# Firstastor/polars-quant

Hardware: AMD Instinct MI355X
Metric: indicator+backtest rows/sec, 5000 sym x 2520 day f64 OHLCV (higher is better)
Workload: dtype f64

## Files before the change

### polars_quant_amd/csrc/fused.hip

```cpp
#include "ops_fused.h"
#include "wt_api.h"

extern "C" {
pq_status pq_trima_chain(pq_ctx *, const pq_batch *, const double *, int64_t, double *);
pq_status pq_cci_chain(pq_ctx *, const pq_batch *, const double *, const double *, const double *, int64_t, double *);
pq_status pq_adxr_chain(pq_ctx *, const pq_batch *, const double *, const double *, const double *, int64_t, double *);
pq_status pq_adxr_from_adx(pq_ctx *, const pq_batch *, const double *, int64_t, double *);
pq_status pq_apo_chain(pq_ctx *, const pq_batch *, const double *, int64_t, int64_t, int64_t, double *);
pq_status pq_ppo_chain(pq_ctx *, const pq_batch *, const double *, int64_t, int64_t, int64_t, double *);
pq_status pq_macdext_chain(pq_ctx *, const pq_batch *, const double *, int64_t, int64_t, int64_t, int64_t, int64_t, int64_t,
                           double *, double *, double *);
pq_status pq_stoch_chain(pq_ctx *, const pq_batch *, const double *, const double *, const double *, int64_t, int64_t,
                         int64_t, int64_t, int64_t, double *, double *);
pq_status pq_stochf_chain(pq_ctx *, const pq_batch *, const double *, const double *, const double *, int64_t, int64_t,
                          int64_t, double *, double *);
pq_status pq_stochrsi_chain(pq_ctx *, const pq_batch *, const double *, int64_t, int64_t, int64_t, int64_t, double *, double *);
}

#define CHK(name, cond) PQ_TRY(pq_check(ctx, b)); PQ_REQUIRE(cond, name ": null pointer")

constexpr int HT_TS_MAX_CHUNKS = 8;
struct HtTsBlob {
    HtAll6Op op;
    const double *real;
// ... 247 lines not shown
    MacdPairOp op{};
    op.a.fast = fast; op.a.slow = slow; op.a.sig = sig; op.b.fast = 12; op.b.slow = 26; op.b.sig = fix_sig;
    InCols<1> in{{real}}; OutCols<6> o{{macd, signal, hist, fmacd, fsignal, fhist}};
    if (PQ_FUSE_OK(ctx) && seq_can_lds(ctx, b, op, in, o)) return launch_seq(ctx, b, op, in, o);
    PQ_TRY(pq_macd(ctx, b, real, fast, slow, sig, macd, signal, hist));
    return pq_macdfix(ctx, b, real, fix_sig, fmacd, fsignal, fhist);
}
pq_status pq_sar_pair(pq_ctx *ctx, const pq_batch *b, const double *high, const double *low, double accel, double maxv, double startvalue,
                      double offsetonreverse, double ai_long, double a_long, double am_long, double ai_short, double a_short,
                      double am_short, double *sar, double *sarext) {
    CHK("pq_sar_pair", high && low && sar && sarext);
    SarPairOp op{};
    op.a.ext = false; op.a.startvalue = 0.0; op.a.offset = 0.0;
    op.a.ai_long = op.a.a_long = op.a.ai_short = op.a.a_short = accel; op.a.am_long = op.a.am_short = maxv;
    op.b.ext = true; op.b.startvalue = startvalue; op.b.offset = offsetonreverse;
    op.b.ai_long = ai_long; op.b.a_long = a_long; op.b.am_long = am_long; op.b.ai_short = ai_short; op.b.a_short = a_short; op.b.am_short = am_short;
    InCols<2> in{{high, low}}; OutCols<2> o{{sar, sarext}};
    if (PQ_FUSE_OK(ctx) && seq_can_lds(ctx, b, op, in, o)) return launch_seq(ctx, b, op, in, o);
    PQ_TRY(pq_sar(ctx, b, high, low, accel, maxv, sar));
    return pq_sarext(ctx, b, high, low, startvalue, offsetonreverse, ai_long, a_long, am_long, ai_short, a_short, am_short, sarext);
}
pq_status pq_volume_all(pq_ctx *ctx, const pq_batch *b, const double *h, const double *l, const double *c, const double *v, int64_t mfi_p,
                        int64_t fast, int64_t slow, double *mfi, double *ad, double *adosc, double *obv) {
    CHK("pq_volume_all", h && l && c && v && mfi && ad && adosc && obv);
    VolumeAllOp op{};
    op.a.p = mfi_p; op.b.a.a.fast = op.b.a.a.slow = 0; op.b.a.b.fast = fast; op.b.a.b.slow = slow;
    InCols<4> in{{h, l, c, v}}; OutCols<4> o{{mfi, ad, adosc, obv}};
    if (PQ_FUSE_OK(ctx) && seq_can_lds(ctx, b, op, in, o)) return launch_seq(ctx, b, op, in, o);
    PQ_TRY(pq_mfi(ctx, b, h, l, c, v, mfi_p, mfi)); PQ_TRY(pq_ad(ctx, b, h, l, c, v, ad));
    PQ_TRY(pq_adosc(ctx, b, h, l, c, v, fast, slow, adosc));
    return pq_obv(ctx, b, c, v, obv);
}
pq_status pq_dm_system_all(pq_ctx *ctx, const pq_batch *b, const double *h, const double *l, const double *c, int64_t p, double *dx,
                           double *plus_di, double *minus_di, double *adx, double *adxr, double *atr, double *natr) {
    CHK("pq_dm_system_all", h && l && c && dx && plus_di && minus_di && adx && adxr && atr && natr);
    {
        pq_status st;
        if (wt_dmi(ctx, b, h, l, c, p, dx, plus_di, minus_di, adx, adxr, &st)) {
            PQ_TRY(st);
            return pq_atr_all(ctx, b, h, l, c, p, atr, natr);
        }
    }
    DmiAtrOp op{}; op.a.p = p; op.b.a.p = p; op.b.b.p = p;
    InCols<3> in{{h, l, c}}; OutCols<7> o{{dx, plus_di, minus_di, adx, adxr, atr, natr}};
    if (PQ_FUSE_OK(ctx) && seq_can_lds(ctx, b, op, in, o)) return launch_seq(ctx, b, op, in, o);
    PQ_TRY(pq_dmi_all(ctx, b, h, l, c, p, dx, plus_di, minus_di, adx, adxr));
    return pq_atr_all(ctx, b, h, l, c, p, atr, natr);
}
pq_status pq_sma_ma(pq_ctx *ctx, const pq_batch *b, const double *real, int64_t p, double *sma, double *ma) {
    CHK("pq_sma_ma", real && sma && ma);
    SmaDupOp op{}; op.a.p = p;
    InCols<1> in{{real}}; OutCols<2> o{{sma, ma}};
    if (PQ_FUSE_OK(ctx) && seq_can_lds(ctx, b, op, in, o)) return launch_seq(ctx, b, op, in, o);
    PQ_TRY(pq_sma(ctx, b, real, p, sma));
    return pq_ma(ctx, b, real, p, 0, ma);
}
pq_status pq_cmo_rsi(pq_ctx *ctx, const pq_batch *b, const double *real, int64_t p, double *cmo, double *rsi) {
    CHK("pq_cmo_rsi", real && cmo && rsi);
    {
        pq_status st;
        if (wt_rsi(ctx, b, real, p, rsi, &st)) { PQ_TRY(st); return pq_cmo(ctx, b, real, p, cmo); }
    }
    CmoRsiOp op{}; op.a.p = p; op.b.p = p;
    InCols<1> in{{real}}; OutCols<2> o{{cmo, rsi}};
    if (PQ_FUSE_OK(ctx) && seq_can_lds(ctx, b, op, in, o)) return launch_seq(ctx, b, op, in, o);
    PQ_TRY(pq_cmo(ctx, b, real, p, cmo));
    return pq_rsi(ctx, b, real, p, rsi);
}
pq_status pq_stoch_all(pq_ctx *ctx, const pq_batch *b, const double *h, const double *l, const double *c, int64_t fastk, int64_t slowk,
                       int64_t slowk_mt, int64_t slowd, int64_t slowd_mt, int64_t fastd, int64_t fastd_mt, double *slowk_out,
                       double *slowd_out, double *fastk_out, double *fastd_out) {
    CHK("pq_stoch_all", h && l && c && slowk_out && slowd_out && fastk_out && fastd_out);
    StochAllOp op{};
    op.fastk = fastk; op.slowk = slowk; op.slowk_mt = slowk_mt; op.slowd = slowd; op.slowd_mt = slowd_mt; op.fastd = fastd; op.fastd_mt = fastd_mt;
    InCols<3> in{{h, l, c}}; OutCols<4> o{{slowk_out, slowd_out, fastk_out, fastd_out}};
    if (PQ_FUSE_OK(ctx) && Ma2::supports(slowk_mt) && Ma2::supports(slowd_mt) && Ma2::supports(fastd_mt) && seq_can_lds(ctx, b, op, in, o))
        return launch_seq(ctx, b, op, in, o);
    PQ_TRY(pq_stoch(ctx, b, h, l, c, fastk, slowk, slowk_mt, slowd, slowd_mt, slowk_out, slowd_out));
    return pq_stochf(ctx, b, h, l, c, fastk, fastd, fastd_mt, fastk_out, fastd_out);
}
pq_status pq_apo_ppo(pq_ctx *ctx, const pq_batch *b, const double *real, int64_t fast, int64_t slow, int64_t matype, double *apo, double *ppo) {
    CHK("pq_apo_ppo", real && apo && ppo);
    ApoPpoOp op{};
    op.a.fast = fast; op.a.slow = slow; op.a.matype = matype; op.b.fast = fast; op.b.slow = slow; op.b.matype = matype;
    InCols<1> in{{real}}; OutCols<2> o{{apo, ppo}};
    if (PQ_FUSE_OK(ctx) && Ma2::supports(matype) && seq_can_lds(ctx, b, op, in, o)) return launch_seq(ctx, b, op, in, o);
    PQ_TRY(pq_apo(ctx, b, real, fast, slow, matype, apo));
    return pq_ppo(ctx, b, real, fast, slow, matype, ppo);
}

}
```

### polars_quant_amd/csrc/ops_fused.h

```cpp
#pragma once
#include "ops_misc.h"
#include "ops_momentum.h"
#include "ops_overlap.h"

struct Ma2 {
    int kind;
    int dead;
    int64_t p, count;
    double k;
    double acc;
    Ring w;
    __host__ __device__ static bool supports(int64_t matype) { return !(matype >= 2 && matype <= 6) && matype != 8; }
    __host__ __device__ static int64_t slots(int64_t matype, int64_t p) { return matype == 1 ? 0 : (p > 0 ? p : 1); }
    __device__ __forceinline__ void init_core(int kind_, int64_t p_, int64_t n) {
        kind = kind_;
        p = p_;
        dead = (p <= 0 || n < p) ? 1 : 0;
        k = pq_uniform(kind ? 2.0 / ((double)p + 1.0) : 1.0 / (double)p);
        count = 0;
        acc = 0.0;
    }
    __device__ __forceinline__ void init(int64_t matype, int64_t p_, int64_t n, RingAlloc &ra) {
        init_core(matype == 1 ? 1 : 0, p_, n);
        if (!kind) w = ra.make(p_);
    }
    __device__ __forceinline__ bool steady() const { return !dead && count >= p; }
    __device__ __forceinline__ double step_old(double v, double old) {
        if (wave_all(!dead && count >= p && !pq_isnull(v))) {
            acc += v;
            acc -= old;
            return acc * k;
        }
        if (dead || pq_isnull(v)) return pq_null();
        count += 1;
        acc += v;
        if (count < p) return pq_null();
        if (count > p) {
            acc -= old;
            count -= 1;
        }
        return acc * k;
    }
    __device__ __forceinline__ double fast_old(double v, double old) {
        acc += v;
        acc -= old;
        return acc * k;
    }
    __device__ __forceinline__ double step(double v) {
        if (!kind) {
            if (wave_all(!dead && count >= p && !pq_isnull(v))) {
                acc += v;
                acc -= w.swap(v);
                return acc * k;
            }
            if (dead || pq_isnull(v)) return pq_null();
            count += 1;
            acc += v;
            const double old = w.swap(v);
            if (count < p) return pq_null();
            if (count > p) {
                acc -= old;
                count -= 1;
            }
            return acc * k;
        }
        if (wave_all(!dead && count >= p && !pq_isnull(v))) {
            acc = fma(k, v - acc, acc);
            return acc;
        }
        if (dead || pq_isnull(v)) return pq_null();
        count += 1;
        if (count < p) {
            acc += v;
            return pq_null();
        } else if (count == p) {
            acc += v;
            acc = acc / (double)p;
            return acc;
        }
        acc = fma(k, v - acc, acc);
        return acc;
    }
    __device__ __forceinline__ double fast(double v) {
        if (!kind) {
            acc += v;
            acc -= w.swap(v);
            return acc * k;
        }
        acc = fma(k, v - acc, acc);
        return acc;
    }
};

struct Ma2Pair {
    Ma2 a, b;
    Ring w;
    bool shared;
    int pa, pb;
    __host__ __device__ static int64_t slots(int64_t mta, int64_t pa_, int64_t mtb, int64_t pb_) {
        if (mta != 1 && mtb != 1) { int64_t m = pa_ > pb_ ? pa_ : pb_; return m > 0 ? m : 1; }
        return Ma2::slots(mta, pa_) + Ma2::slots(mtb, pb_);
    }
    __device__ __forceinline__ void init(int64_t mta, int64_t pa_, int64_t mtb, int64_t pb_, int64_t n, RingAlloc &ra) {
        shared = (mta != 1 && mtb != 1);
        if (shared) {
            a.init_core(0, pa_, n); b.init_core(0, pb_, n);
            pa = (int)(pa_ > 0 ? pa_ : 1); pb = (int)(pb_ > 0 ? pb_ : 1);
            w = ra.make(pa_ > pb_ ? pa_ : pb_);
            asm volatile("" ::: "memory");
        } else {
            a.init(mta, pa_, n, ra); b.init(mtb, pb_, n, ra);
        }
    }
    __device__ __forceinline__ void step(double v, double &ya, double &yb) {
        if (!shared) { ya = a.step(v); yb = b.step(v); return; }
        if (pq_isnull(v)) { ya = yb = pq_null(); return; }
        const double oa = w.get(pa), ob = w.get(pb);
        ya = a.step_old(v, oa);
        yb = b.step_old(v, ob);
        w.push(v);
    }
    __device__ __forceinline__ bool steady() const { return a.steady() && b.steady(); }
    __device__ __forceinline__ void fast(double v, double &ya, double &yb) {
        if (!shared) { ya = a.fast(v); yb = b.fast(v); return; }
        const double oa = w.get(pa), ob = w.get(pb);
        ya = a.fast_old(v, oa);
        yb = b.fast_old(v, ob);
        w.push(v);
    }
};

struct TrimaOp {
    static constexpr bool LDS_ONLY = true;
    static constexpr int NIN = 1, NOUT = 1;
    static constexpr int SEQ_ID = 70;
    static constexpr int COST_NS = 150;
    int64_t k1, k2;
    SmaCore a, b;
    Ring wa, wb;
    __host__ __device__ int64_t ring_slots() const { return (k1 > 0 ? k1 : 1) + (k2 > 0 ? k2 : 1); }
    __device__ void init(const Row<1> &) {}
    __device__ void init_lds(const Row<1> &r, RingAlloc &ra) { a.init(k1, r.len); b.init(k2, r.len); wa = ra.make(k1); wb = ra.make(k2); }
    __device__ void step(const Row<1> &, int64_t, const double (&)[1], double (&y)[1]) { y[0] = pq_null(); }
    __device__ void step_lds(int64_t, const double (&x)[1], double (&y)[1]) { y[0] = b.step_ring(wb, a.step_ring(wa, x[0])); }
    static constexpr bool HAS_FAST = true;
    __device__ bool steady(int64_t) const { return a.steady() && b.steady(); }
    __device__ void step_fast(int64_t, const double (&x)[1], double (&y)[1]) { y[0] = b.fast_ring(wb, a.fast_ring(wa, x[0])); }
};

struct SmaDupOp {
    static constexpr bool LDS_ONLY = true;
    static constexpr int NIN = 1, NOUT = 2;
    static constexpr int SEQ_ID = 88;
    static constexpr int ASSIST = 1;
    static constexpr int ALG_COLS = 4;
    static constexpr int COST_NS = 130;
    SmaOp a;
    __host__ __device__ int64_t ring_slots() const { return a.ring_slots(); }
    __device__ void init(const Row<1> &) {}
    __device__ void init_lds(const Row<1> &r, RingAlloc &ra) { a.init_lds(r, ra); }
    __device__ void step(const Row<1> &, int64_t, const double (&)[1], double (&y)[2]) { y[0] = y[1] = pq_null(); }
    __device__ void step_lds(int64_t t, const double (&x)[1], double (&y)[2]) { double v[1]; a.step_lds(t, x, v); y[0] = y[1] = v[0]; }
    static constexpr bool HAS_FAST = true;
    __device__ bool steady(int64_t t0) const { return a.steady(t0); }
    __device__ void step_fast(int64_t t, const double (&x)[1], double (&y)[2]) { double v[1]; a.step_fast(t, x, v); y[0] = y[1] = v[0]; }
    static constexpr bool FAST_BATCH = true;
    static constexpr int FAST_UNROLL = 8;
    template <int N>
    __device__ void steps_fast(int64_t t, const double (&x)[N][1], double (&y)[N][2]) {
        double v[N][1];
        a.template steps_fast<N>(t, x, v);
#pragma unroll
        for (int u = 0; u < N; u++) y[u][0] = y[u][1] = v[u][0];
    }
};

template <int MODE>
struct MaDiffOp {
    static constexpr bool LDS_ONLY = true;
    static constexpr int NIN = 1, NOUT = 1;
    static constexpr int SEQ_ID = 71 + MODE;
    static constexpr int COST_NS = 500;
    int64_t fast, slow, matype;
    Ma2Pair fs;
    __host__ __device__ int64_t ring_slots() const { return Ma2Pair::slots(matype, fast, matype, slow); }
    __device__ void init(const Row<1> &) {}
    __device__ void init_lds(const Row<1> &r, RingAlloc &ra) { fs.init(matype, fast, matype, slow, r.len, ra); }
    __device__ void step(const Row<1> &, int64_t, const double (&)[1], double (&y)[1]) { y[0] = pq_null(); }
    __device__ void step_lds(int64_t, const double (&x)[1], double (&y)[1]) {
        double a, b;
        fs.step(x[0], a, b);
        if (pq_isnull(a) || pq_isnull(b)) { y[0] = pq_null(); return; }
        if (MODE == 0) y[0] = a - b;
        else y[0] = (b == 0.0) ? pq_null() : (a - b) / b * 100.0;
    }
    static constexpr bool HAS_FAST = true;
    __device__ bool steady(int64_t) const { return fs.steady(); }
    __device__ void step_fast(int64_t, const double (&x)[1], double (&y)[1]) {
        double a, b;
        fs.fast(x[0], a, b);
        if (MODE == 0) y[0] = a - b;
        else { const double v = (a - b) / b * 100.0; y[0] = (b == 0.0) ? pq_null() : v; }
    }
};

struct MacdextOp {
    static constexpr bool LDS_ONLY = true;
    static constexpr int NIN = 1, NOUT = 3;
    static constexpr int SEQ_ID = 73;
    static constexpr int COST_NS = 338;
    int64_t fast, fastmt, slow, slowmt, sig, sigmt;
    Ma2Pair fs;
    Ma2 g;
    __host__ __device__ int64_t ring_slots() const { return Ma2Pair::slots(fastmt, fast, slowmt, slow) + Ma2::slots(sigmt, sig); }
    __device__ __forceinline__ void init(const Row<1> &) {}
    __device__ __forceinline__ void init_lds(const Row<1> &r, RingAlloc &ra) {
        fs.init(fastmt, fast, slowmt, slow, r.len, ra); g.init(sigmt, sig, r.len, ra);
    }
    __device__ __forceinline__ void step(const Row<1> &, int64_t, const double (&)[1], double (&y)[3]) { y[0] = y[1] = y[2] = pq_null(); }
    __device__ __forceinline__ void step_lds(int64_t, const double (&x)[1], double (&y)[3]) {
        double a, b;
        fs.step(x[0], a, b);
        double m = (pq_isnull(a) || pq_isnull(b)) ? pq_null() : a - b;
        double d = g.step(m);
        y[0] = m; y[1] = d;
        y[2] = (pq_isnull(m) || pq_isnull(d)) ? pq_null() : m - d;
    }
    static constexpr bool HAS_FAST = true;
    __device__ __forceinline__ bool steady(int64_t) const { return fs.steady() && g.steady(); }
    __device__ __forceinline__ void step_fast(int64_t, const double (&x)[1], double (&y)[3]) {
        double a, b;
        fs.fast(x[0], a, b);
        const double m = a - b;
        const double d = g.fast(m);
        y[0] = m; y[1] = d; y[2] = m - d;
    }
};

struct FastkCore {
    int64_t k, rows, nulls_h, nulls_l;
    Ring nh, nl;
    RollExt<true> mx;
    RollExt<false> mn;
    Ring hc, hs, lc, ls;
    __host__ __device__ static int64_t slots(int64_t k) { return 6 * (k > 0 ? k : 1); }
    __device__ void init(int64_t k_, RingAlloc &ra) {
        k = k_; rows = 0; nulls_h = nulls_l = 0;
        nh = ra.make(k); nl = ra.make(k);
        mx.init(k); mn.init(k); mx.init_ring(); mn.init_ring();
        hc = ra.make(k); hs = ra.make(k); lc = ra.make(k); ls = ra.make(k);
    }
    __device__ double step(double h, double l, double c) {
        if (k <= 0) return pq_null();
        const bool hn_ = pq_isnull(h), ln_ = pq_isnull(l);
        double oh = nh.swap(hn_ ? 1.0 : 0.0), ol = nl.swap(ln_ ? 1.0 : 0.0);
        if (rows >= k) { nulls_h -= (oh != 0.0) ? 1 : 0; nulls_l -= (ol != 0.0) ? 1 : 0; }
        nulls_h += hn_ ? 1 : 0; nulls_l += ln_ ? 1 : 0;
        rows += 1;
        double hmax = mx.step_ring2(hc, hs, hn_ ? -1.7976931348623157e308 : h);
        double lmin = mn.step_ring2(lc, ls, ln_ ? 1.7976931348623157e308 : l);
        if (rows < k || nulls_h || nulls_l || pq_isnull(c)) return pq_null();
        return (c - lmin) * 100.0 / (hmax - lmin);
    }
    __device__ bool steady() const { return k > 0 && rows >= k && nulls_h == 0 && nulls_l == 0; }
    __device__ double fast(double h, double l, double c) {
        const double hmax = mx.step_ring2(hc, hs, h);
        const double lmin = mn.step_ring2(lc, ls, l);
        return (c - lmin) * 100.0 / (hmax - lmin);
    }
};

template <int MODE>
struct StochOp {
    static constexpr bool RG_GATHER = true;
    static constexpr int64_t DIRECT_LANE_MAX = 16384;
    static constexpr bool LDS_ONLY = true;
    static constexpr int NIN = 3, NOUT = 2;
    static constexpr int SEQ_ID = 74 + MODE;
    static constexpr int COST_NS = MODE == 0 ? 637 : 579;
    static constexpr bool HEAVY = false;
    int64_t fastk, p1, mt1, p2, mt2;
    FastkCore fk;
    Ma2 m1, m2;
    __host__ __device__ int64_t ring_slots() const {
        return FastkCore::slots(fastk) + Ma2::slots(mt1, p1) + (MODE == 0 ? Ma2::slots(mt2, p2) : 0);
    }
    __device__ void init(const Row<3> &) {}
    __device__ void init_lds(const Row<3> &r, RingAlloc &ra) {
        fk.init(fastk, ra);
        m1.init(mt1, p1, r.len, ra);
        if (MODE == 0) m2.init(mt2, p2, r.len, ra);
    }
    __device__ void step(const Row<3> &, int64_t, const double (&)[3], double (&y)[2]) { y[0] = y[1] = pq_null(); }
    __device__ void step_lds(int64_t, const double (&x)[3], double (&y)[2]) {
        double k = fk.step(x[0], x[1], x[2]);
        double a = m1.step(k);
        if (MODE == 0) { y[0] = a; y[1] = m2.step(a); }
        else { y[0] = k; y[1] = a; }
    }
    static constexpr bool HAS_FAST = true;
    __device__ bool steady(int64_t) const { return fk.steady() && m1.steady() && (MODE != 0 || m2.steady()); }
    __device__ void step_fast(int64_t, const double (&x)[3], double (&y)[2]) {
        const double k = fk.fast(x[0], x[1], x[2]);
        const double a = m1.fast(k);
        if (MODE == 0) { y[0] = a; y[1] = m2.fast(a); }
        else { y[0] = k; y[1] = a; }
    }
};

struct StochAllOp {
    static constexpr bool RG_GATHER = true;
    static constexpr bool LDS_ONLY = true;
    static constexpr int NIN = 3, NOUT = 4;
    static constexpr int ALG_COLS = 5 + 5;
    static constexpr int SEQ_ID = 96;
    static constexpr int COST_NS = 800;
    int64_t fastk, slowk, slowk_mt, slowd, slowd_mt, fastd, fastd_mt;
    FastkCore fk;
    Ma2 mk, md, mf;
    __host__ __device__ int64_t ring_slots() const {
        return FastkCore::slots(fastk) + Ma2::slots(slowk_mt, slowk) + Ma2::slots(slowd_mt, slowd) + Ma2::slots(fastd_mt, fastd);
    }
    __device__ void init(const Row<3> &) {}
    __device__ void init_lds(const Row<3> &r, RingAlloc &ra) {
        fk.init(fastk, ra);
        mk.init(slowk_mt, slowk, r.len, ra); md.init(slowd_mt, slowd, r.len, ra); mf.init(fastd_mt, fastd, r.len, ra);
    }
    __device__ void step(const Row<3> &, int64_t, const double (&)[3], double (&y)[4]) { y[0] = y[1] = y[2] = y[3] = pq_null(); }
    __device__ void step_lds(int64_t, const double (&x)[3], double (&y)[4]) {
        const double k = fk.step(x[0], x[1], x[2]);
        const double a = mk.step(k);
        y[0] = a; y[1] = md.step(a); y[2] = k; y[3] = mf.step(k);
    }
    static constexpr bool HAS_FAST = true;
    __device__ bool steady(int64_t) const { return fk.steady() && mk.steady() && md.steady() && mf.steady(); }
    __device__ void step_fast(int64_t, const double (&x)[3], double (&y)[4]) {
        const double k = fk.fast(x[0], x[1], x[2]);
        const double a = mk.fast(k);
        y[0] = a; y[1] = md.fast(a); y[2] = k; y[3] = mf.fast(k);
    }
};

struct StochRsiOp {
    static constexpr bool RG_GATHER = true;
    static constexpr int64_t DIRECT_LANE_MAX = 16384;
    static constexpr bool LDS_ONLY = true;
    static constexpr int NIN = 1, NOUT = 2;
    static constexpr int SEQ_ID = 76;
    static constexpr int COST_NS = 618;
    int64_t p, fastk, fastd, fastd_mt;
    RsiOp rsi;
    FastkCore fk;
    Ma2 m;
    __host__ __device__ int64_t ring_slots() const { return FastkCore::slots(fastk) + Ma2::slots(fastd_mt, fastd); }
    __device__ void init(const Row<1> &) {}
    __device__ void init_lds(const Row<1> &r, RingAlloc &ra) { rsi.p = p; rsi.init(r); fk.init(fastk, ra); m.init(fastd_mt, fastd, r.len, ra); }
    __device__ void step(const Row<1> &, int64_t, const double (&)[1], double (&y)[2]) { y[0] = y[1] = pq_null(); }
    __device__ void step_lds(int64_t i, const double (&x)[1], double (&y)[2]) {
        double rv[1];
        Row<1> dummy; dummy.in[0] = nullptr; dummy.len = 0;
        rsi.step(dummy, i, x, rv);
        double k = fk.step(rv[0], rv[0], rv[0]);
        y[0] = k;
        y[1] = m.step(k);
    }
    static constexpr bool FAST_NULL_OK = true;
    static constexpr bool HAS_FAST = true;
    __device__ bool steady(int64_t t0) const { return rsi.steady(t0) && fk.steady() && m.steady(); }
    __device__ void step_fast(int64_t i, const double (&x)[1], double (&y)[2]) {
        double rv[1];
        rsi.step_fast(i, x, rv);
        const double k = fk.fast(rv[0], rv[0], rv[0]);
        y[0] = k;
        y[1] = m.fast(k);
    }
};

struct CciOp {
    static constexpr bool LDS_ONLY = true;
    static constexpr int NIN = 3, NOUT = 1;
    static constexpr int SEQ_ID = 77;
    __host__ int cost_ns() const { return 320 + 40 * (int)(p > 0 ? (p < 1000 ? p : 1000) : 0); }
    int64_t p;
    double sum, denom;
    bool dead;
    Ring w;
    __host__ __device__ int64_t ring_slots() const { return p > 0 ? p : 1; }
    __device__ void init(const Row<3> &) {}
    __device__ void init_lds(const Row<3> &r, RingAlloc &ra) {
        dead = (p <= 0 || r.len < p); sum = 0.0; denom = 1.0 / (double)p; w = ra.make(p);
    }
    __device__ void step(const Row<3> &, int64_t, const double (&)[3], double (&y)[1]) { y[0] = pq_null(); }
    __device__ void step_lds(int64_t i, const double (&x)[3], double (&y)[1]) {
        y[0] = pq_null();
        if (dead) return;
        double tp = (x[0] + x[1] + x[2]) / 3.0;
        sum += tp;
        double old = w.swap(tp);
        if (i < p - 1) return;
        if (i >= p) sum -= old;
        double avg = sum * denom;
        double mean_dev = 0.0;
        for (int b0 = (int)p; b0 >= 1; b0 -= 8) {
            double v8[8];
            w.get8<-1>(b0, v8);
#pragma unroll
            for (int u = 0; u < 8; u++)
                if (b0 - u >= 1) mean_dev += fabs(v8[u] - avg);
        }
        if (mean_dev != 0.0) {
            mean_dev /= (double)p;
            y[0] = (tp - avg) / (0.015 * mean_dev);
        }
    }
    static constexpr bool FAST_NULL_OK = true;
    static constexpr bool HAS_FAST = true;
    __device__ bool steady(int64_t t0) const { return !dead && t0 >= p; }
    __device__ void step_fast(int64_t, const double (&x)[3], double (&y)[1]) {
        const double tp = (x[0] + x[1] + x[2]) / 3.0;
        sum += tp;
        sum -= w.swap(tp);
        const double avg = sum * denom;
        double mean_dev = 0.0;
        for (int b0 = (int)p; b0 >= 1; b0 -= 8) {
            double v8[8];
            w.get8<-1>(b0, v8);
#pragma unroll
            for (int u = 0; u < 8; u++)
                if (b0 - u >= 1) mean_dev += fabs(v8[u] - avg);
        }
        const double md = mean_dev / (double)p;
        const double v = (tp - avg) / (0.015 * md);
        y[0] = (mean_dev != 0.0) ? v : pq_null();
    }
    static constexpr bool FAST_BATCH = true;
    static constexpr int FAST_UNROLL = 8;
    template <int N>
    __device__ void steps_fast(int64_t, const double (&x)[N][3], double (&y)[N][1]) {
        static_assert(N == 8, "CciOp::steps_fast is written for batches of eight rows");
        double tp[8], old[8], avg[8], md[8];
#pragma unroll
        for (int r = 0; r < 8; r++) tp[r] = (x[r][0] + x[r][1] + x[r][2]) / 3.0;
        w.swap_n<8>(tp, old);
#pragma unroll
        for (int r = 0; r < 8; r++) {
            sum += tp[r];
            sum -= old[r];
            avg[r] = sum * denom;
            md[r] = 0.0;
        }
        double W[15];
#pragma unroll
        for (int i = 0; i < 7; i++) W[i] = old[i + 1];
        int k = w.pos;
        const int ip = (int)p;
        for (int b0 = 0; b0 < ip; b0 += 8) {
#pragma unroll
// ... 432 lines not shown
template <int ID, class A, class B>
struct Fuse2 {
    static_assert(A::NIN == B::NIN, "fused ops must read the same input columns");
    static_assert(!IsMasked<A>::value && !IsMasked<B>::value && !HasFinish<A>::value && !HasFinish<B>::value, "not fusable");
    static_assert(NTap<A>::value == 0 || HasRings<A>::value, "tap-only ops cannot be fused");
    static_assert(NTap<B>::value == 0 || HasRings<B>::value, "tap-only ops cannot be fused");
    static constexpr int NIN = A::NIN, NOUT = A::NOUT + B::NOUT;
    static constexpr int ALG_COLS = AlgCols<A>::value + AlgCols<B>::value;
    static constexpr int SEQ_ID = ID;
    static constexpr int ASSIST = FuseAssist<ID>::value;
    __host__ int cost_ns() const { return (3 * (OpCost<A>::get(a) + OpCost<B>::get(b))) / 4; }
    static constexpr bool HEAVY = IsHeavy<A>::value || IsHeavy<B>::value;
    static constexpr bool LDS_ONLY = true;
    A a;
    B b;
    __host__ __device__ int64_t ring_slots() const {
        int64_t n = 0;
        if constexpr (HasRings<A>::value) n += a.ring_slots();
        if constexpr (HasRings<B>::value) n += b.ring_slots();
        return n;
    }
    __device__ void init(const Row<NIN> &) {}
    __device__ void init_lds(const Row<NIN> &r, RingAlloc &ra) {
        if constexpr (HasRings<A>::value) a.init_lds(r, ra); else a.init(r);
        if constexpr (HasRings<B>::value) b.init_lds(r, ra); else b.init(r);
        row = r;
    }
    Row<NIN> row;
    __device__ void step(const Row<NIN> &, int64_t, const double (&)[NIN], double (&y)[NOUT]) {
#pragma unroll
        for (int k = 0; k < NOUT; k++) y[k] = pq_null();
    }
    __device__ void step_lds(int64_t t, const double (&x)[NIN], double (&y)[NOUT]) {
        double ya[A::NOUT], yb[B::NOUT];
        if constexpr (HasRings<A>::value) a.step_lds(t, x, ya); else a.step(row, t, x, ya);
        if constexpr (HasRings<B>::value) b.step_lds(t, x, yb); else b.step(row, t, x, yb);
#pragma unroll
        for (int k = 0; k < A::NOUT; k++) y[k] = ya[k];
#pragma unroll
        for (int k = 0; k < B::NOUT; k++) y[A::NOUT + k] = yb[k];
    }
    static constexpr bool FAST_NULL_OK = FastNullOk<A>::value && FastNullOk<B>::value;
    static constexpr int FAST_UNROLL = FastUnroll<A>::value < FastUnroll<B>::value ? FastUnroll<A>::value : FastUnroll<B>::value;
    static constexpr bool HAS_FAST = HasFast<A>::value && HasFast<B>::value;
    __device__ bool steady(int64_t t0) const { return a.steady(t0) && b.steady(t0); }
    __device__ void step_fast(int64_t t, const double (&x)[NIN], double (&y)[NOUT]) {
        double ya[A::NOUT], yb[B::NOUT];
        a.step_fast(t, x, ya);
        b.step_fast(t, x, yb);
#pragma unroll
        for (int k = 0; k < A::NOUT; k++) y[k] = ya[k];
#pragma unroll
        for (int k = 0; k < B::NOUT; k++) y[A::NOUT + k] = yb[k];
    }
};

template <int NIN_, class Op, int I0, int I1>
struct Pick2 {
    static_assert(Op::NIN == 2 && !HasRings<Op>::value && NTap<Op>::value == 0, "Pick2 wraps a plain two-input op");
    static constexpr int NIN = NIN_, NOUT = Op::NOUT;
    static constexpr int ALG_COLS = AlgCols<Op>::value;
    static constexpr int COST_NS = OpCostStatic<Op>::value;
    Op op;
    Row<2> rr;
    __device__ void init(const Row<NIN> &r) { rr.in[0] = r.in[I0]; rr.in[1] = r.in[I1]; rr.len = r.len; op.init(rr); }
    __device__ void step(const Row<NIN> &, int64_t t, const double (&x)[NIN], double (&y)[NOUT]) {
        const double xx[2] = {x[I0], x[I1]};
        op.step(rr, t, xx, y);
    }
    static constexpr bool FAST_NULL_OK = FastNullOk<Op>::value;
    static constexpr bool HAS_FAST = HasFast<Op>::value;
    __device__ bool steady(int64_t t0) const { return op.steady(t0); }
    __device__ void step_fast(int64_t t, const double (&x)[NIN], double (&y)[NOUT]) {
        const double xx[2] = {x[I0], x[I1]};
        op.step_fast(t, xx, y);
    }
};

typedef Fuse2<90, Fuse2<0, EmaOp, DemaOp>, Fuse2<0, TemaOp, TrixOp>> EmaAllOp;
typedef Fuse2<91, AtrOp<false>, AtrOp<true>> AtrAllOp;
typedef Fuse2<92, DmRawOp<true>, DmRawOp<false>> DmPairOp;
typedef Fuse2<93, AdOp<false>, AdOp<true>> AdAllOp;
typedef Fuse2<94, MacdOp, MacdOp> MacdPairOp;
typedef Fuse2<95, MaDiffOp<0>, MaDiffOp<1>> ApoPpoOp;
typedef Fuse2<97, SarextOp, SarextOp> SarPairOp;
typedef Fuse2<99, DmAllOp<true>, AtrAllOp> DmiAtrOp;
typedef Fuse2<89, CmoOp, RsiOp> CmoRsiOp;
typedef Fuse2<98, MfiOp, Fuse2<0, AdAllOp, Pick2<4, ObvOp, 2, 3>>> VolumeAllOp;
```

### polars_quant_amd/csrc/ops_overlap.h

```cpp
#pragma once
#include "pq_cores.h"

struct SmaOp {
    static constexpr int NIN = 1, NOUT = 1;
    static constexpr int SEQ_ID = 1;
    static constexpr int COST_NS = 116;
    static constexpr int NTAP = 1;
    static constexpr int TAP_COL[1] = {0};
    int64_t p;
    SmaCore c;
    __device__ void init(const Row<1> &r) { c.init(p, r.len); }
    __device__ void tap_lags(int64_t (&lag)[1]) const { lag[0] = c.dead ? 0 : p; }
    __device__ void step(const Row<1> &r, int64_t t, const double (&x)[1], const double (&tp)[1], double (&y)[1]) {
        y[0] = c.step(r.in[0], t, x[0], tp[0]);
    }
    Ring w;
    __host__ __device__ int64_t ring_slots() const { return p > 0 ? p : 1; }
    __device__ void init_lds(const Row<1> &r, RingAlloc &ra) { c.init(p, r.len); w = ra.make(p); }
    __device__ void step_lds(int64_t, const double (&x)[1], double (&y)[1]) { y[0] = c.step_ring(w, x[0]); }
    static constexpr bool HAS_FAST = true;
    __device__ bool steady(int64_t) const { return c.steady(); }
    __device__ void step_fast(int64_t, const double (&x)[1], double (&y)[1]) { y[0] = c.fast_ring(w, x[0]); }
    static constexpr bool FAST_BATCH = true;
    static constexpr int FAST_UNROLL = 16;
// ... 381 lines not shown
    }
    Ring w;
    __host__ __device__ int64_t ring_slots() const { return p > 0 ? 2 * p : 1; }
    __device__ void init_lds(const Row<1> &r, RingAlloc &ra) { init(r); w = ra.make(2 * p); }
    __device__ void step_lds(int64_t, const double (&x)[1], double (&y)[1]) {
        y[0] = pq_null();
        double v = x[0];
        if (dead || pq_isnull(v)) return;
        if (count == 0) { count = 1; x0 = v; j = 1; w.push(v); return; }
        if (count < p) { count += 1; sum += fabs(v - x0); j += 1; w.push(v); return; }
        int64_t k = j - p + 1;
        double xa = w.get((int)p), xk = w.get((int)p - 1);
        double diff_abs = fabs(v - xa);
        double popped = (k < p) ? fabs(xk - x0) : fabs(xk - w.get((int)(2 * p - 1)));
        sum += diff_abs - popped;
        double er = diff_abs / sum;
        j += 1;
        w.push(v);
        double sc_sqrt = er * (2.0 / 3.0 - 2.0 / 31.0) + 2.0 / 31.0;
        double sc = sc_sqrt * sc_sqrt;
        if (c2 < p) { c2 += 1; sum2 += v; return; }
        if (c2 == p) { c2 += 1; kama = sum2 / (double)p; y[0] = kama; return; }
        kama = fma(sc, v - kama, kama);
        y[0] = kama;
    }
    static constexpr bool HAS_FAST = true;
    __device__ bool steady(int64_t) const { return !dead && count >= p && j >= 2 * p - 1 && c2 > p; }
    __device__ void step_fast(int64_t, const double (&x)[1], double (&y)[1]) {
        const double v = x[0];
        const double xa = w.get((int)p), xk = w.get((int)p - 1), xc = w.get((int)(2 * p - 1));
        double diff_abs = fabs(v - xa);
        double popped = fabs(xk - xc);
        sum += diff_abs - popped;
        double er = diff_abs / sum;
        w.push(v);
        double sc_sqrt = er * (2.0 / 3.0 - 2.0 / 31.0) + 2.0 / 31.0;
        double sc = sc_sqrt * sc_sqrt;
        kama = fma(sc, v - kama, kama);
        y[0] = kama;
    }
};

struct MidpointOp {
    static constexpr int NIN = 1, NOUT = 1;
    static constexpr int SEQ_ID = 9;
    static constexpr int COST_NS = 246;
    int64_t p;
    RollExt<true> mx;
    double mn;
    bool any, frozen;
    const double *col;
    __device__ void init(const Row<1> &r) { mx.init(p); mn = 0.0; any = false; frozen = false; col = r.in[0]; }
    __device__ __forceinline__ void low(double v) {
        if (!any) { mn = v; any = true; }
        else if (!frozen && v <= mn) mn = v;
        frozen |= v != v;
    }
    __device__ void step(const Row<1> &r, int64_t t, const double (&x)[1], double (&y)[1]) {
        double v = x[0];
        if (p <= 0 || pq_isnull(v)) { y[0] = pq_null(); return; }
        double m = mx.nan_row(r.in[0], t, v, mx.step(r.in[0], t, v));
        low(v);
        y[0] = (m + mn) / 2.0;
    }
    Ring wc, ws;
    __host__ __device__ int64_t ring_slots() const { return p > 0 ? 2 * p : 2; }
    __device__ void init_lds(const Row<1> &r, RingAlloc &ra) { init(r); mx.init_ring(); wc = ra.make(p); ws = ra.make(p); }
    __device__ void step_lds(int64_t t, const double (&x)[1], double (&y)[1]) {
        double v = x[0];
        if (p <= 0 || pq_isnull(v)) { y[0] = pq_null(); return; }
        double m = mx.nan_row(col, t, v, mx.step_ring2(wc, ws, v));
        low(v);
        y[0] = (m + mn) / 2.0;
    }
    static constexpr bool HAS_FAST = true;
    __device__ bool steady(int64_t) const { return p > 0 && any; }
    __device__ void step_fast(int64_t t, const double (&x)[1], double (&y)[1]) {
        const double v = x[0];
        const double m = mx.nan_row(col, t, v, mx.step_ring2(wc, ws, v));
        mn = (!frozen && v <= mn) ? v : mn;
        frozen |= v != v;
        y[0] = (m + mn) / 2.0;
    }
};

struct MidpriceOp {
    static constexpr int NIN = 2, NOUT = 1;
    static constexpr int SEQ_ID = 10;
    static constexpr int COST_NS = 416;
    int64_t p;
    RollExt<true> mx;
    RollExt<false> mn;
    const double *ch, *cl;
    __device__ void init(const Row<2> &r) { mx.init(p); mn.init(p); ch = r.in[0]; cl = r.in[1]; }
    __device__ void step(const Row<2> &r, int64_t t, const double (&x)[2], double (&y)[1]) {
        double hm = pq_null(), lm = pq_null();
        if (p <= 0) { y[0] = pq_null(); return; }
        if (!pq_isnull(x[0])) hm = mx.nan_row(r.in[0], t, x[0], mx.step(r.in[0], t, x[0]));
        if (!pq_isnull(x[1])) lm = mn.nan_row(r.in[1], t, x[1], mn.step(r.in[1], t, x[1]));
        y[0] = (pq_isnull(hm) || pq_isnull(lm)) ? pq_null() : (hm + lm) / 2.0;
    }
    Ring whc, whs, wlc, wls;
    __host__ __device__ int64_t ring_slots() const { return p > 0 ? 4 * p : 4; }
    __device__ void init_lds(const Row<2> &r, RingAlloc &ra) {
        init(r); mx.init_ring(); mn.init_ring();
        whc = ra.make(p); whs = ra.make(p); wlc = ra.make(p); wls = ra.make(p);
    }
    __device__ void step_lds(int64_t t, const double (&x)[2], double (&y)[1]) {
        if (p <= 0) { y[0] = pq_null(); return; }
        double hm = pq_null(), lm = pq_null();
        if (!pq_isnull(x[0])) hm = mx.nan_row(ch, t, x[0], mx.step_ring2(whc, whs, x[0]));
        if (!pq_isnull(x[1])) lm = mn.nan_row(cl, t, x[1], mn.step_ring2(wlc, wls, x[1]));
        y[0] = (pq_isnull(hm) || pq_isnull(lm)) ? pq_null() : (hm + lm) / 2.0;
    }
    static constexpr bool HAS_FAST = true;
    __device__ bool steady(int64_t) const { return p > 0; }
    __device__ void step_fast(int64_t t, const double (&x)[2], double (&y)[1]) {
        const double hm = mx.nan_row(ch, t, x[0], mx.step_ring2(whc, whs, x[0]));
        const double lm = mn.nan_row(cl, t, x[1], mn.step_ring2(wlc, wls, x[1]));
        y[0] = (hm + lm) / 2.0;
    }
};

struct MidpriceRowOp {
    static constexpr int NIN = 2, NOUT = 1;
    static constexpr int ROW_ID = 18;
    typedef double OutT;
    int64_t p;
    __device__ void eval(const Row<2> &r, int64_t t, double (&y)[1]) {
        y[0] = pq_null();
        if (p <= 0) return;
        const double h0 = r.in[0][t], l0 = r.in[1][t];
        if (pq_isnull(h0) || pq_isnull(l0)) return;
        y[0] = (roll_ext_ref<true>(r.in[0], t, p) + roll_ext_ref<false>(r.in[1], t, p)) / 2.0;
    }
};

__device__ __forceinline__ double n0(double x) { return pq_isnull(x) ? 0.0 : x; }

struct SarextOp {
    static constexpr bool RG_GATHER = true;
    static constexpr int64_t DIRECT_LANE_MAX = 16384;
    static constexpr int NIN = 2, NOUT = 1;
    static constexpr int SEQ_ID = 11;
    static constexpr int COST_NS = 450;
    bool ext;
    double startvalue, offset, ai_long, a_long, am_long, ai_short, a_short, am_short;
    double af_long, af_short, ep, sar, new_low, new_high;
    bool is_long;
    __device__ void init(const Row<2> &r) {
        af_long = ai_long; af_short = ai_short;
        if (af_long > am_long) af_long = ai_long = am_long;
        if (a_long > am_long) a_long = am_long;
        if (af_short > am_short) af_short = ai_short = am_short;
        if (a_short > am_short) a_short = am_short;
        if (r.len < 2) return;
        double h0 = n0(r.in[0][0]), l0 = n0(r.in[1][0]), h1 = n0(r.in[0][1]), l1 = n0(r.in[1][1]);
        if (startvalue == 0.0) {
            double diffP = h1 - h0, diffM = l0 - l1;
            is_long = !(diffM > 0.0 && diffP < diffM);
            if (is_long) { ep = h1; sar = l0; } else { ep = l1; sar = h0; }
        } else if (startvalue > 0.0) { is_long = true; ep = h1; sar = startvalue; }
        else { is_long = false; ep = l1; sar = fabs(startvalue); }
        new_low = l1; new_high = h1;
    }
    __device__ void step(const Row<2> &r, int64_t t, const double (&x)[2], double (&y)[1]) {
        y[0] = pq_null();
        if (r.len < 2 || t == 0) return;
        row(x, y);
    }
    static constexpr bool HAS_FAST = true;
    static constexpr bool FAST_NULL_OK = true;
    __device__ bool steady(int64_t t0) const { return t0 >= 1; }
    __device__ void step_fast(int64_t, const double (&x)[2], double (&y)[1]) { row(x, y); }
    __device__ __forceinline__ void row(const double (&x)[2], double (&y)[1]) {
        double prev_low = new_low, prev_high = new_high;
        new_high = n0(x[0]); new_low = n0(x[1]);
        if (is_long) {
            if (new_low <= sar) {
                is_long = false; sar = ep;
                if (sar < prev_high) sar = prev_high;
                if (sar < new_high) sar = new_high;
                if (ext && offset != 0.0) sar += sar * offset;
                y[0] = ext ? -sar : sar;
                af_short = ai_short; ep = new_low;
                sar = sar + af_short * (ep - sar);
                if (sar < prev_high) sar = prev_high;
                if (sar < new_high) sar = new_high;
            } else {
                y[0] = sar;
                if (new_high > ep) { ep = new_high; af_long += a_long; if (af_long > am_long) af_long = am_long; }
                sar = sar + af_long * (ep - sar);
                if (sar > prev_low) sar = prev_low;
                if (sar > new_low) sar = new_low;
            }
        } else {
            if (new_high >= sar) {
                is_long = true; sar = ep;
                if (sar > prev_low) sar = prev_low;
                if (sar > new_low) sar = new_low;
                if (ext && offset != 0.0) sar -= sar * offset;
                y[0] = sar;
                af_long = ai_long; ep = new_high;
// ... 98 lines not shown
```

### polars_quant_amd/csrc/pq_cores.h

```cpp
#pragma once
#include "pq_dev.h"

__device__ __forceinline__ bool wave_all(bool x) { return __builtin_amdgcn_ballot_w64(x) == __builtin_amdgcn_ballot_w64(true); }
__device__ __forceinline__ double pq_uniform(double x) {
    const int lo = __builtin_amdgcn_readfirstlane(__double2loint(x)), hi = __builtin_amdgcn_readfirstlane(__double2hiint(x));
    return __hiloint2double(hi, lo);
}

struct EmaCore {
    int64_t p, count;
    double alpha, ema, sum;
    bool dead;
    __device__ void init(int64_t p_, int64_t n) {
        p = p_;
        dead = (p <= 0 || n < p);
        alpha = pq_uniform(2.0 / ((double)p + 1.0));
        count = 0;
        ema = 0.0;
        sum = 0.0;
    }
    __device__ double step(double v) {
        if (wave_all(!dead && count >= p && !pq_isnull(v))) {
            ema = fma(alpha, v - ema, ema);
            return ema;
// ... 164 lines not shown
__device__ __forceinline__ double roll_ext_ref(const double *col, int64_t t, int64_t p) {
    double run = 0.0;
    bool have = false;
    int64_t cnt = 0;
    for (int64_t i = t; i >= 0 && cnt < p; i--) {
        const double w = col[i];
        if (pq_isnull(w)) continue;
        cnt++;
        if (w != w) have = false;
        else if (!have || (IS_MAX ? w > run : w < run)) { run = w; have = true; }
    }
    return have ? run : __longlong_as_double(0x7FF8000000000000LL);
}
template <bool IS_MAX>
struct RollExt {
    int64_t p, j;
    double best;
    int64_t best_j;
    Regular reg;
    int64_t nan_left;
    __device__ void init(int64_t p_) {
        p = p_;
        j = 0;
        best = 0.0;
        best_j = 0;
        nan_left = 0;
        reg.init();
    }
    __device__ __forceinline__ double nan_row(const double *col, int64_t t, double v, double m) {
        if (v != v) nan_left = p;
        if (nan_left > 0) { nan_left -= 1; m = roll_ext_ref<IS_MAX>(col, t, p); }
        return m;
    }
    __device__ static bool beats(double a, double b) { return IS_MAX ? (a >= b) : (a <= b); }
    __device__ double step(const double *col, int64_t t, double v) {
        bool regular = reg.push(t);
        j += 1;
        if (j == 1 || beats(v, best)) {
            best = v;
            best_j = j;
        } else if (p > 0 && best_j == j - p) {
            best = v;
            best_j = j;
            if (regular) {
                int64_t k = 1;
                for (; k + 8 <= p; k += 8) {
                    double w[8];
#pragma unroll
                    for (int u = 0; u < 8; u++) w[u] = col[t - k - u];
#pragma unroll
                    for (int u = 0; u < 8; u++)
                        if (IS_MAX ? (w[u] > best) : (w[u] < best)) { best = w[u]; best_j = j - k - u; }
                }
                for (; k < p; k++) {
                    double w = col[t - k];
                    if (IS_MAX ? (w > best) : (w < best)) { best = w; best_j = j - k; }
                }
            } else {
                int64_t jj = j, i = t;
                for (int64_t k = 1; k < p; k++) {
                    do { i--; } while (pq_isnull(col[i]));
                    jj--;
                    double w = col[i];
                    if (IS_MAX ? (w > best) : (w < best)) { best = w; best_j = jj; }
                }
            }
        }
        return best;
    }
    int64_t m;
    bool has_prev;
    double prefix;
    __device__ void init_ring() { m = 0; has_prev = false; prefix = 0.0; }
    __device__ double step_ring2(Ring &cur, Ring &suf, double v) {
        if (p <= 0) return v;
        prefix = (m == 0) ? v : (IS_MAX ? fmax(prefix, v) : fmin(prefix, v));
        cur.base[m * 64] = v;
        m += 1;
        double out = prefix;
        if (has_prev && m < p) {
            double s = suf.base[m * 64];
            out = IS_MAX ? fmax(out, s) : fmin(out, s);
        }
        if (m == p) {
            double run = cur.base[(p - 1) * 64];
            suf.base[(p - 1) * 64] = run;
            for (int64_t k = p - 2; k >= 0; k--) {
                double x = cur.base[k * 64];
                run = IS_MAX ? fmax(run, x) : fmin(run, x);
                suf.base[k * 64] = run;
            }
            m = 0;
            has_prev = true;
        }
        return out;
    }
};
```

Measured before the change: 3.853 billion.

## Batch steady-state steps for MA, stochastic and rolling extremum fused ops

Adds unrolled multi-step fast paths (steps_fast/fast_n) for Ma2, Ma2Pair, MA-diff, MACDEXT, stochastic variants, midpoint/midprice, and a batched ring-based rolling max/min with wave-uniform block position. It replaces the generic Fuse2 APO/PPO with a dedicated op that shares one MA pair, and lets stoch_all reuse the slow-K average when the fast-D parameters match. The aim is to cut per-step LDS traffic and loop overhead and to drop redundant averages. In exchange it adds register pressure and a fragile index path that falls back when lanes disagree.

```diff
diff --git a/polars_quant_amd/csrc/fused.hip b/polars_quant_amd/csrc/fused.hip
--- a/polars_quant_amd/csrc/fused.hip
+++ b/polars_quant_amd/csrc/fused.hip
@@ -353,7 +353,7 @@
 pq_status pq_apo_ppo(pq_ctx *ctx, const pq_batch *b, const double *real, int64_t fast, int64_t slow, int64_t matype, double *apo, double *ppo) {
     CHK("pq_apo_ppo", real && apo && ppo);
     ApoPpoOp op{};
-    op.a.fast = fast; op.a.slow = slow; op.a.matype = matype; op.b.fast = fast; op.b.slow = slow; op.b.matype = matype;
+    op.fast = fast; op.slow = slow; op.matype = matype;
     InCols<1> in{{real}}; OutCols<2> o{{apo, ppo}};
     if (PQ_FUSE_OK(ctx) && Ma2::supports(matype) && seq_can_lds(ctx, b, op, in, o)) return launch_seq(ctx, b, op, in, o);
     PQ_TRY(pq_apo(ctx, b, real, fast, slow, matype, apo));
diff --git a/polars_quant_amd/csrc/ops_fused.h b/polars_quant_amd/csrc/ops_fused.h
--- a/polars_quant_amd/csrc/ops_fused.h
+++ b/polars_quant_amd/csrc/ops_fused.h
@@ -90,6 +90,18 @@
         acc = fma(k, v - acc, acc);
         return acc;
     }
+    template <int N>
+    __device__ __forceinline__ void fast_n(const double (&v)[N], double (&y)[N]) {
+        if (!kind) {
+            double old[N];
+            w.swap_n<N>(v, old);
+#pragma unroll
+            for (int u = 0; u < N; u++) { acc += v[u]; acc -= old[u]; y[u] = acc * k; }
+        } else {
+#pragma unroll
+            for (int u = 0; u < N; u++) { acc = fma(k, v[u] - acc, acc); y[u] = acc; }
+        }
+    }
 };
 
 struct Ma2Pair {
@@ -127,6 +139,21 @@
         ya = a.fast_old(v, oa);
         yb = b.fast_old(v, ob);
         w.push(v);
+    }
+    template <int N>
+    __device__ __forceinline__ void fast_n(const double (&v)[N], double (&ya)[N], double (&yb)[N]) {
+        if (!shared) { a.template fast_n<N>(v, ya); b.template fast_n<N>(v, yb); return; }
+        if (pa < N || pb < N) {
+#pragma unroll
+            for (int u = 0; u < N; u++) fast(v[u], ya[u], yb[u]);
+            return;
+        }
+        double oa[N], ob[N];
+#pragma unroll
+        for (int u = 0; u < N; u++) { oa[u] = w.get(pa - u); ob[u] = w.get(pb - u); }
+        w.push_n<N>(v);
+#pragma unroll
+        for (int u = 0; u < N; u++) { ya[u] = a.fast_old(v[u], oa[u]); yb[u] = b.fast_old(v[u], ob[u]); }
     }
 };
 
@@ -202,6 +229,65 @@
         if (MODE == 0) y[0] = a - b;
         else { const double v = (a - b) / b * 100.0; y[0] = (b == 0.0) ? pq_null() : v; }
     }
+    static constexpr bool FAST_BATCH = true;
+    static constexpr int FAST_UNROLL = 8;
+    template <int N>
+    __device__ void steps_fast(int64_t, const double (&x)[N][1], double (&y)[N][1]) {
+        double v[N], a[N], b[N];
+#pragma unroll
+        for (int u = 0; u < N; u++) v[u] = x[u][0];
+        fs.template fast_n<N>(v, a, b);
+#pragma unroll
+        for (int u = 0; u < N; u++) {
+            if (MODE == 0) y[u][0] = a[u] - b[u];
+            else { const double q = pq_keep((a[u] - b[u]) / b[u] * 100.0); y[u][0] = (b[u] == 0.0) ? pq_null() : q; }
+        }
+    }
+};
+
+struct ApoPpoOp {
+    static constexpr bool LDS_ONLY = true;
+    static constexpr int NIN = 1, NOUT = 2;
+    static constexpr int ALG_COLS = 2 + 2;
+    static constexpr int SEQ_ID = 95;
+    static constexpr int COST_NS = 750;
+    int64_t fast, slow, matype;
+    Ma2Pair fs;
+    __host__ __device__ int64_t ring_slots() const { return Ma2Pair::slots(matype, fast, matype, slow); }
+    __device__ void init(const Row<1> &) {}
+    __device__ void init_lds(const Row<1> &r, RingAlloc &ra) { fs.init(matype, fast, matype, slow, r.len, ra); }
+    __device__ void step(const Row<1> &, int64_t, const double (&)[1], double (&y)[2]) { y[0] = y[1] = pq_null(); }
+    __device__ void step_lds(int64_t, const double (&x)[1], double (&y)[2]) {
+        double a, b;
+        fs.step(x[0], a, b);
+        if (pq_isnull(a) || pq_isnull(b)) { y[0] = y[1] = pq_null(); return; }
+        y[0] = a - b;
+        y[1] = (b == 0.0) ? pq_null() : (a - b) / b * 100.0;
+    }
+    static constexpr bool HAS_FAST = true;
+    __device__ bool steady(int64_t) const { return fs.steady(); }
+    __device__ void step_fast(int64_t, const double (&x)[1], double (&y)[2]) {
+        double a, b;
+        fs.fast(x[0], a, b);
+        const double d = a - b, q = pq_keep(d / b * 100.0);
+        y[0] = d;
+        y[1] = (b == 0.0) ? pq_null() : q;
+    }
+    static constexpr bool FAST_BATCH = true;
+    static constexpr int FAST_UNROLL = 8;
+    template <int N>
+    __device__ void steps_fast(int64_t, const double (&x)[N][1], double (&y)[N][2]) {
+        double v[N], a[N], b[N];
+#pragma unroll
+        for (int u = 0; u < N; u++) v[u] = x[u][0];
+        fs.template fast_n<N>(v, a, b);
+#pragma unroll
+        for (int u = 0; u < N; u++) {
+            const double d = a[u] - b[u], q = pq_keep(d / b[u] * 100.0);
+            y[u][0] = d;
+            y[u][1] = (b[u] == 0.0) ? pq_null() : q;
+        }
+    }
 };
 
 struct MacdextOp {
@@ -234,6 +320,20 @@
         const double m = a - b;
         const double d = g.fast(m);
         y[0] = m; y[1] = d; y[2] = m - d;
+    }
+    static constexpr bool FAST_BATCH = true;
+    static constexpr int FAST_UNROLL = 8;
+    template <int N>
+    __device__ __forceinline__ void steps_fast(int64_t, const double (&x)[N][1], double (&y)[N][3]) {
+        double v[N], a[N], b[N], m[N], d[N];
+#pragma unroll
+        for (int u = 0; u < N; u++) v[u] = x[u][0];
+        fs.template fast_n<N>(v, a, b);
+#pragma unroll
+        for (int u = 0; u < N; u++) m[u] = a[u] - b[u];
+        g.template fast_n<N>(m, d);
+#pragma unroll
+        for (int u = 0; u < N; u++) { y[u][0] = m[u]; y[u][1] = d[u]; y[u][2] = m[u] - d[u]; }
     }
 };
 
@@ -268,6 +368,22 @@
         const double lmin = mn.step_ring2(lc, ls, l);
         return (c - lmin) * 100.0 / (hmax - lmin);
     }
+    template <int N>
+    __device__ __forceinline__ void fast_n(const double (&h)[N], const double (&l)[N], const double (&c)[N], double (&y)[N]) {
+        double hmax[N], lmin[N];
+        if (mx.template steps_ok<N>() && mn.template steps_ok<N>()) {
+            mx.template steps_ring2<N>(hc, hs, h, hmax);
+            mn.template steps_ring2<N>(lc, ls, l, lmin);
+        } else {
+#pragma unroll
+            for (int u = 0; u < N; u++) {
+                hmax[u] = mx.step_ring2(hc, hs, h[u]);
+                lmin[u] = mn.step_ring2(lc, ls, l[u]);
+            }
+        }
+#pragma unroll
+        for (int u = 0; u < N; u++) y[u] = (c[u] - lmin[u]) * 100.0 / (hmax[u] - lmin[u]);
+    }
 };
 
 template <int MODE>
@@ -306,6 +422,22 @@
         if (MODE == 0) { y[0] = a; y[1] = m2.fast(a); }
         else { y[0] = k; y[1] = a; }
     }
+    static constexpr bool FAST_BATCH = true;
+    static constexpr int FAST_UNROLL = 4;
+    template <int N>
+    __device__ void steps_fast(int64_t, const double (&x)[N][3], double (&y)[N][2]) {
+        double h[N], l[N], c[N], k[N], a[N], d[N];
+#pragma unroll
+        for (int u = 0; u < N; u++) { h[u] = x[u][0]; l[u] = x[u][1]; c[u] = x[u][2]; }
+        fk.template fast_n<N>(h, l, c, k);
+        m1.template fast_n<N>(k, a);
+        if (MODE == 0) m2.template fast_n<N>(a, d);
+#pragma unroll
+        for (int u = 0; u < N; u++) {
+            if (MODE == 0) { y[u][0] = a[u]; y[u][1] = d[u]; }
+            else { y[u][0] = k[u]; y[u][1] = a[u]; }
+        }
+    }
 };
 
 struct StochAllOp {
@@ -318,26 +450,47 @@
     int64_t fastk, slowk, slowk_mt, slowd, slowd_mt, fastd, fastd_mt;
     FastkCore fk;
     Ma2 mk, md, mf;
+    __host__ __device__ bool one_avg() const { return slowk == fastd && slowk_mt == fastd_mt; }
     __host__ __device__ int64_t ring_slots() const {
-        return FastkCore::slots(fastk) + Ma2::slots(slowk_mt, slowk) + Ma2::slots(slowd_mt, slowd) + Ma2::slots(fastd_mt, fastd);
+        return FastkCore::slots(fastk) + Ma2::slots(slowk_mt, slowk) + Ma2::slots(slowd_mt, slowd) + (one_avg() ? 0 : Ma2::slots(fastd_mt, fastd));
     }
     __device__ void init(const Row<3> &) {}
     __device__ void init_lds(const Row<3> &r, RingAlloc &ra) {
         fk.init(fastk, ra);
-        mk.init(slowk_mt, slowk, r.len, ra); md.init(slowd_mt, slowd, r.len, ra); mf.init(fastd_mt, fastd, r.len, ra);
+        mk.init(slowk_mt, slowk, r.len, ra); md.init(slowd_mt, slowd, r.len, ra);
+        if (!one_avg()) mf.init(fastd_mt, fastd, r.len, ra);
     }
     __device__ void step(const Row<3> &, int64_t, const double (&)[3], double (&y)[4]) { y[0] = y[1] = y[2] = y[3] = pq_null(); }
     __device__ void step_lds(int64_t, const double (&x)[3], double (&y)[4]) {
         const double k = fk.step(x[0], x[1], x[2]);
         const double a = mk.step(k);
-        y[0] = a; y[1] = md.step(a); y[2] = k; y[3] = mf.step(k);
-    }
-    static constexpr bool HAS_FAST = true;
-    __device__ bool steady(int64_t) const { return fk.steady() && mk.steady() && md.steady() && mf.steady(); }
+        y[0] = a; y[1] = md.step(a); y[2] = k; y[3] = one_avg() ? a : mf.step(k);
+    }
+    static constexpr bool HAS_FAST = true;
+    __device__ bool steady(int64_t) const { return fk.steady() && mk.steady() && md.steady() && (one_avg() || mf.steady()); }
     __device__ void step_fast(int64_t, const double (&x)[3], double (&y)[4]) {
         const double k = fk.fast(x[0], x[1], x[2]);
         const double a = mk.fast(k);
-        y[0] = a; y[1] = md.fast(a); y[2] = k; y[3] = mf.fast(k);
+        y[0] = a; y[1] = md.fast(a); y[2] = k; y[3] = one_avg() ? a : mf.fast(k);
+    }
+    static constexpr bool FAST_BATCH = true;
+    static constexpr int FAST_UNROLL = 4;
+    template <int N>
+    __device__ void steps_fast(int64_t, const double (&x)[N][3], double (&y)[N][4]) {
+        double h[N], l[N], c[N], k[N], a[N], d[N], f[N];
+#pragma unroll
+        for (int u = 0; u < N; u++) { h[u] = x[u][0]; l[u] = x[u][1]; c[u] = x[u][2]; }
+        fk.template fast_n<N>(h, l, c, k);
+        mk.template fast_n<N>(k, a);
+        md.template fast_n<N>(a, d);
+        if (one_avg()) {
+#pragma unroll
+            for (int u = 0; u < N; u++) f[u] = a[u];
+        } else {
+            mf.template fast_n<N>(k, f);
+        }
+#pragma unroll
+        for (int u = 0; u < N; u++) { y[u][0] = a[u]; y[u][1] = d[u]; y[u][2] = k[u]; y[u][3] = f[u]; }
     }
 };
 
@@ -373,6 +526,22 @@
         const double k = fk.fast(rv[0], rv[0], rv[0]);
         y[0] = k;
         y[1] = m.fast(k);
+    }
+    static constexpr bool FAST_BATCH = true;
+    static constexpr int FAST_UNROLL = 4;
+    template <int N>
+    __device__ void steps_fast(int64_t i, const double (&x)[N][1], double (&y)[N][2]) {
+        double rv[N], k[N], d[N];
+#pragma unroll
+        for (int u = 0; u < N; u++) {
+            double r1[1];
+            rsi.step_fast(i + u, x[u], r1);
+            rv[u] = r1[0];
+        }
+        fk.template fast_n<N>(rv, rv, rv, k);
+        m.template fast_n<N>(k, d);
+#pragma unroll
+        for (int u = 0; u < N; u++) { y[u][0] = k[u]; y[u][1] = d[u]; }
     }
 };
 
@@ -971,7 +1140,6 @@
 typedef Fuse2<92, DmRawOp<true>, DmRawOp<false>> DmPairOp;
 typedef Fuse2<93, AdOp<false>, AdOp<true>> AdAllOp;
 typedef Fuse2<94, MacdOp, MacdOp> MacdPairOp;
-typedef Fuse2<95, MaDiffOp<0>, MaDiffOp<1>> ApoPpoOp;
 typedef Fuse2<97, SarextOp, SarextOp> SarPairOp;
 typedef Fuse2<99, DmAllOp<true>, AtrAllOp> DmiAtrOp;
 typedef Fuse2<89, CmoOp, RsiOp> CmoRsiOp;
diff --git a/polars_quant_amd/csrc/ops_overlap.h b/polars_quant_amd/csrc/ops_overlap.h
--- a/polars_quant_amd/csrc/ops_overlap.h
+++ b/polars_quant_amd/csrc/ops_overlap.h
@@ -487,6 +487,26 @@
         frozen |= v != v;
         y[0] = (m + mn) / 2.0;
     }
+    static constexpr bool FAST_BATCH = true;
+    static constexpr int FAST_UNROLL = 4;
+    template <int N>
+    __device__ void steps_fast(int64_t t, const double (&x)[N][1], double (&y)[N][1]) {
+        double v[N], m[N];
+        bool nan = mx.nan_left > 0;
+#pragma unroll
+        for (int u = 0; u < N; u++) { v[u] = x[u][0]; nan |= v[u] != v[u]; }
+        if (wave_all(!nan) && mx.template steps_ok<N>()) {
+            mx.template steps_ring2<N>(wc, ws, v, m);
+#pragma unroll
+            for (int u = 0; u < N; u++) {
+                mn = (!frozen && v[u] <= mn) ? v[u] : mn;
+                y[u][0] = (m[u] + mn) / 2.0;
+            }
+            return;
+        }
+#pragma unroll
+        for (int u = 0; u < N; u++) step_fast(t + u, x[u], y[u]);
+    }
 };
 
 struct MidpriceOp {
@@ -524,6 +544,24 @@
         const double hm = mx.nan_row(ch, t, x[0], mx.step_ring2(whc, whs, x[0]));
         const double lm = mn.nan_row(cl, t, x[1], mn.step_ring2(wlc, wls, x[1]));
         y[0] = (hm + lm) / 2.0;
+    }
+    static constexpr bool FAST_BATCH = true;
+    static constexpr int FAST_UNROLL = 4;
+    template <int N>
+    __device__ void steps_fast(int64_t t, const double (&x)[N][2], double (&y)[N][1]) {
+        double h[N], l[N], hm[N], lm[N];
+        bool nan = mx.nan_left > 0 || mn.nan_left > 0;
+#pragma unroll
+        for (int u = 0; u < N; u++) { h[u] = x[u][0]; l[u] = x[u][1]; nan |= h[u] != h[u] || l[u] != l[u]; }
+        if (wave_all(!nan) && mx.template steps_ok<N>() && mn.template steps_ok<N>()) {
+            mx.template steps_ring2<N>(whc, whs, h, hm);
+            mn.template steps_ring2<N>(wlc, wls, l, lm);
+#pragma unroll
+            for (int u = 0; u < N; u++) y[u][0] = (hm[u] + lm[u]) / 2.0;
+            return;
+        }
+#pragma unroll
+        for (int u = 0; u < N; u++) step_fast(t + u, x[u], y[u]);
     }
 };
 
diff --git a/polars_quant_amd/csrc/pq_cores.h b/polars_quant_amd/csrc/pq_cores.h
--- a/polars_quant_amd/csrc/pq_cores.h
+++ b/polars_quant_amd/csrc/pq_cores.h
@@ -270,17 +270,61 @@
             double s = suf.base[m * 64];
             out = IS_MAX ? fmax(out, s) : fmin(out, s);
         }
-        if (m == p) {
-            double run = cur.base[(p - 1) * 64];
-            suf.base[(p - 1) * 64] = run;
-            for (int64_t k = p - 2; k >= 0; k--) {
-                double x = cur.base[k * 64];
-                run = IS_MAX ? fmax(run, x) : fmin(run, x);
-                suf.base[k * 64] = run;
+        if (m == p) finish_block(cur, suf);
+        return out;
+    }
+    __device__ static double ext(double a, double b) { return IS_MAX ? fmax(a, b) : fmin(a, b); }
+    static constexpr int BURST = 4;
+    __device__ __forceinline__ void finish_block(Ring &cur, Ring &suf) {
+        double run = 0.0;
+        for (int64_t k0 = p - 1; k0 >= 0; k0 -= BURST) {
+            double xb[BURST];
+#pragma unroll
+            for (int u = 0; u < BURST; u++) xb[u] = cur.base[(k0 - u >= 0 ? k0 - u : 0) * 64];
+#pragma unroll
+            for (int u = 0; u < BURST; u++)
+                if (k0 - u >= 0) {
+                    run = (k0 - u == p - 1) ? xb[u] : ext(run, xb[u]);
+                    suf.base[(k0 - u) * 64] = run;
+                }
+        }
+        m = 0;
+        has_prev = true;
+    }
+    template <int N>
+    __device__ __forceinline__ bool steps_ok() const {
+        return wave_all(has_prev && p >= N && (int)m == __builtin_amdgcn_readfirstlane((int)m));
+    }
+    template <int N>
+    __device__ __forceinline__ void steps_ring2(Ring &cur, Ring &suf, const double (&v)[N], double (&out)[N]) {
+        const int ms = __builtin_amdgcn_readfirstlane((int)m), ps = __builtin_amdgcn_readfirstlane((int)p);
+        const int uc = ps - 1 - ms;
+        double s[N];
+#pragma unroll
+        for (int u = 0; u < N; u++) {
+            const int i = ms + u + 1;
+            s[u] = suf.base[(i < ps ? i : ps - 1) * 64];
+        }
+#pragma unroll
+        for (int u = 0; u < N; u++)
+            if (u <= uc) cur.base[(ms + u) * 64] = v[u];
+        if (uc < N) {
+            finish_block(cur, suf);
+#pragma unroll
+            for (int u = 1; u < N; u++)
+                if (u > uc) cur.base[(u - uc - 1) * 64] = v[u];
+#pragma unroll
+            for (int u = 1; u < N; u++) {
+                const double t = suf.base[(u > uc ? u - uc : 0) * 64];
+                s[u] = (u > uc) ? t : s[u];
             }
-            m = 0;
-            has_prev = true;
-        }
-        return out;
-    }
-};
+        }
+#pragma unroll
+        for (int u = 0; u < N; u++) {
+            const int mb = (u <= uc) ? ms + u : u - uc - 1;
+            prefix = (mb == 0) ? v[u] : ext(prefix, v[u]);
+            out[u] = (u == uc) ? prefix : ext(prefix, s[u]);
+        }
+        m = (uc < N) ? N - 1 - uc : ms + N;
+    }
+};
```

New measurement: 3.920 billion (median of 6 runs). 1.7% higher.
